# Darkkey/erlamsa

Measured on AMD Instinct MI355X. Metric: mutated_MB_per_s, higher is better.
Workload: dtype u8 (byte edits) + f64 (AS183 draws)

## Files before the change

erlamsa_amd/csrc/eh_device.h:

```cpp
#pragma once
#include <hip/hip_runtime.h>
#include <stdint.h>

#include "eh_common.h"

namespace eh {

#define EH_LANE ((int)threadIdx.x)
#define EH_DEV __device__ __forceinline__

EH_DEV uint32_t uni(uint32_t v) { return (uint32_t)__builtin_amdgcn_readfirstlane((int)v); }
EH_DEV uint64_t uni64(uint64_t v) { return ((uint64_t)uni((uint32_t)(v >> 32)) << 32) | uni((uint32_t)v); }
EH_DEV void wave_sync() { __syncthreads(); }

struct alignas(16) TabU16x65 { uint16_t v[65]; };
constexpr TabU16x65 as183_powers(uint32_t mult, uint32_t prime) {
  TabU16x65 t{};
  uint32_t a = 1;
  for (int k = 0; k <= 64; k++) { t.v[k] = (uint16_t)a; a = a * mult % prime; }
  return t;
}
__constant__ TabU16x65 c_T1 = as183_powers(171, 30269);
__constant__ TabU16x65 c_T2 = as183_powers(172, 30307);
__constant__ TabU16x65 c_T3 = as183_powers(170, 30323);
// ... 238 lines not shown
  bptr trace;
  uint32_t ntrace, tr_base;
  uint32_t co_posted;
  int32_t call_req, mu_phase, call_nres, call_nfs;
  uint64_t call_bin; uint32_t call_len;
  EH_G MuFrame* mu;
  uint64_t t_case;
  int32_t m_aux;
  uint64_t ws_peak, ws_top;
  int status;
  int lastm;
  uint64_t work;
  int r_kind;
  bptr r_ptr;
  uint32_t r_len;
  int r_flush;
  int r_drop_next;
  int r_changed;
  int r2; bptr r2_ptr; uint32_t r2_len;
  int nfs;
  uint64_t work_budget;
  uint64_t ovf_need, ovf_req;
  int ovf_line;
  int depth;
  int gen_pending;
  uint32_t gen_e1, gen_e2;
  int pat_ret; uint32_t pat_ip; int pat_cont;
  uint32_t fp_on, fp_g, fp_special, fp_keypos, fp_bA, fp_bB;
};
__shared__ Ctx g_ctx;
#ifdef HIPEMU
#define EH_LDS_ARRAY(type, name, n) static type name[n]
#define EH_KEEP(v) do {} while (0)
#else
#define EH_LDS_ARRAY(type, name, n) __shared__ type name[n]
#define EH_KEEP(v) asm volatile("" : "+v"(v))
#endif
EH_DEV void lanes_sync() { (void)__ballot(1); }
#define EH_CTX Ctx& c = g_ctx
#ifndef EH_FUSE_LDS_WORDS
#define EH_FUSE_LDS_WORDS 4800
#endif
EH_LDS_ARRAY(uint32_t, g_fuse_lds, EH_FUSE_LDS_WORDS);
EH_LDS_ARRAY(uint32_t, g_st_save, ST_STATE_WORDS);
struct LaneTab {
  uint32_t e_pri;
  uint32_t e_meta;
};
enum { R_SAME = 0, R_NEW = 1 };

#ifdef EH_PROF
#define EH_PT0 uint64_t pt_ = __builtin_readcyclecounter()
#define EH_PT(c, k) do { uint64_t n_ = __builtin_readcyclecounter(); if (EH_LANE == 0) { atomicAdd(&(c).p->prof[2 * (k)], (unsigned long long)(n_ - pt_)); atomicAdd(&(c).p->prof[2 * (k) + 1], 1ull); } pt_ = n_; } while (0)
#else
#define EH_PT0 do {} while (0)
#define EH_PT(c, k) do {} while (0)
#endif

EH_DEV void tr_b(Ctx& c, uint32_t v) {
  if (c.ntrace < TRACE_CAP - 1) { if (EH_LANE == 0) c.trace[c.ntrace] = (uint8_t)v; c.ntrace++; }
  else { if (EH_LANE == 0) c.trace[TRACE_CAP - 1] = 0xFF; c.ntrace = TRACE_CAP; }
}
EH_DEV void tr_v(Ctx& c, uint64_t v) { while (v >= 128) { tr_b(c, (uint32_t)(v & 127u) | 128u); v >>= 7; } tr_b(c, (uint32_t)v); }
__device__ __noinline__ void tr_aa_emit(int a, int b) { Ctx& c = g_ctx; tr_b(c, TRK_AA); tr_b(c, (uint32_t)a); tr_b(c, (uint32_t)b); }
__device__ __noinline__ void tr_ai_emit(int a, int64_t v) { Ctx& c = g_ctx; tr_b(c, TRK_AI); tr_b(c, (uint32_t)a); tr_v(c, ((uint64_t)v << 1) ^ (uint64_t)(v >> 63)); }
__device__ __noinline__ void tr_kv_emit(int kind, int nb, uint32_t b0, uint32_t b1, int nv, uint64_t v0, uint64_t v1, uint64_t v2) {
  Ctx& c = g_ctx;
  tr_b(c, (uint32_t)kind);
  if (nb > 0) tr_b(c, b0);
  if (nb > 1) tr_b(c, b1);
  if (nv > 0) tr_v(c, v0);
  if (nv > 1) tr_v(c, v1);
  if (nv > 2) tr_v(c, v2);
}
__device__ __noinline__ void tr_name_emit(cbptr nm, uint32_t nl, uint32_t up) {
  Ctx& c = g_ctx;
  tr_b(c, TRK_ARCHIVER); tr_v(c, nl + 3u * up);
  for (uint32_t k = 0; k < up; k++) { tr_b(c, '.'); tr_b(c, '.'); tr_b(c, '/'); }
  for (uint32_t k = 0; k < nl; k++) tr_b(c, uni(nm[k]));
}
EH_DEV void tr_aa(Ctx& c, int a, int b) { if (__builtin_expect(c.trace != nullptr, 0)) tr_aa_emit(a, b); }
EH_DEV void tr_ai(Ctx& c, int a, int64_t v) { if (__builtin_expect(c.trace != nullptr, 0)) tr_ai_emit(a, v); }
EH_DEV void tr_drop_before(Ctx& c, uint32_t start) {
  if (!c.trace || start <= c.tr_base || c.ntrace >= TRACE_CAP) return;
  const uint32_t n = c.ntrace - start;
  wave_sync();
  if (n) wave_move_down(c.trace + c.tr_base, c.trace + start, n);
  wave_sync();
  c.ntrace = c.tr_base + n;
}

EH_DEV void pool_nap() {
#ifndef HIPEMU
  __builtin_amdgcn_s_sleep(64);
#else
  fprintf(stderr, "hipemu: a wait for a pool area can never end with one wavefront running (block %u)\n", blockIdx.x); abort();
#endif
}
EH_DEV uint32_t pool_pop(const EH_G KParams& p, int t) {
  uint32_t v = 0xFFFFFFFFu;
  if (EH_LANE == 0) {
    unsigned long long h = atomicAdd(&p.pool_ctr[2 * t], 1ull);
    wptr e = p.pool_ring[t] + (h % p.pool_cnt[t]);
    v = atomicExch(e, 0xFFFFFFFFu);
    if (v == 0xFFFFFFFFu) {
      uint64_t w0 = __builtin_readcyclecounter();
      for (;;) { pool_nap(); v = atomicExch(e, 0xFFFFFFFFu); if (v != 0xFFFFFFFFu) break; }
      atomicAdd(&p.pool_ctr[20 + t], (unsigned long long)(__builtin_readcyclecounter() - w0));
      atomicAdd(&p.pool_ctr[30 + t], 1ull);
// ... 789 lines not shown
```

erlamsa_amd/csrc/eh_fuse.h:

```cpp
#pragma once
#include "eh_field.h"

namespace eh {

struct FNode { uint32_t fo, fc, to, tc; };

EH_DEV uint32_t wave_sort64(uint32_t key) {
  const uint32_t l = (uint32_t)EH_LANE;
#pragma unroll
  for (uint32_t k2 = 2; k2 <= 64; k2 <<= 1) {
#pragma unroll
    for (uint32_t j = k2 >> 1; j > 0; j >>= 1) {
      uint32_t other = (uint32_t)__shfl_xor((int)key, (int)j);
      bool up = (l & k2) == 0 || k2 == 64, lower = (l & j) == 0;
      bool take_min = lower == up;
      uint32_t mn = key < other ? key : other, mx = key < other ? other : key;
      key = take_min ? mn : mx;
    }
  }
  return key;
}
EH_DEV uint32_t lanes_le(uint32_t v, uint32_t cnt, uint32_t x) {
  uint32_t lo = 0;
#pragma unroll
// ... 231 lines not shown
    if (child) {
      FNode c2;
      c2.fc = nf; c2.tc = nt;
      c2.fo = special ? la : (nf == 1 ? fsurv + 1 : of);
      c2.to = special ? lb : (nt == 1 ? tsurv + 1 : (nt == 0 ? 0u : ot));
      o.nd[oc] = c2;
      le += nf + nt;
    }
    {
      bool lmulti = __shfl((int)(child && !special && nf > 1 ? 1 : 0), (int)lead[0]) != 0;
      uint32_t lof = (uint32_t)__shfl((int)of, (int)lead[0]);
      bool ldrop = __shfl((int)(isdrop[0] ? 1 : 0), (int)lead[0]) != 0;
      if (alive[0] && lmulti && !isdrop[0]) o.F[lof + ((uint32_t)l - lead[0]) - (ldrop ? 1u : 0u)] = pos[0] + 1;
    }
    if (!sym) {
      uint32_t sl = lanes_lt(gk[0], totf, gk[1]);
      uint32_t sk_at = (uint32_t)__shfl((int)gk[0], (int)(sl & 63));
      bool has = alive[1] && sl < totf && sk_at == gk[1];
      bool smulti = __shfl((int)(child && !special && nt > 1 ? 1 : 0), (int)(sl & 63)) != 0;
      uint32_t sot = (uint32_t)__shfl((int)ot, (int)(sl & 63));
      bool ldrop = __shfl((int)(isdrop[1] ? 1 : 0), (int)lead[1]) != 0;
      if (has && smulti && !isdrop[1]) o.T[sot + ((uint32_t)l - lead[1]) - (ldrop ? 1u : 0u)] = pos[1] + 1;
    }
    cn += (uint32_t)__builtin_amdgcn_readlane((int)ic, 63); cf += (uint32_t)__builtin_amdgcn_readlane((int)iff, 63); ct += (uint32_t)__builtin_amdgcn_readlane((int)it, 63);
    k0 += nfit;
  }
  *entries = wave_sum64(le);
  wave_sync();
  return cn;
}

__device__ bool fuse_jump_stream(Ctx& c, cbptr A, uint32_t la, cbptr B, uint32_t lb, bool sym, uint32_t* from, uint32_t* tpos, uint32_t* rounds);
}
#include "eh_fuse_red.h"
namespace eh {

#ifdef EH_FUSE_INLINE
EH_DEV bool fuse_lists(Ctx& c, cbptr A, uint32_t la, cbptr B, uint32_t lb, bptr* out, uint32_t* outlen) {
#else
__device__ __noinline__ bool fuse_lists(Ctx&, cbptr A, uint32_t la, cbptr B, uint32_t lb, bptr* out, uint32_t* outlen) {
  EH_CTX;
#endif
  const int l = EH_LANE;
  if (la == 0) { *out = (bptr)B; *outlen = lb; return true; }
  if (lb == 0) { *out = (bptr)A; *outlen = la; return true; }
  uint64_t mark = c.ws_used;
  const bool sym = A == B && la == lb;
  EH_PT0;
  uint32_t from = la, tpos = lb;
  uint32_t prof_rounds = 0;
  c.fp_on = 0;
  if ((sym ? (uint64_t)la : (uint64_t)la + lb) > FL_NMAX && !c.work_budget && !(c.p->flags & EH_FLAG_FUSE_NO_REDUCE)) {
    const uint32_t rd = fr_peek_rounds(c.rng);
    if (rd < 64) {
      const uint32_t R = rd + 2u;
      uint32_t la2 = la, lb2 = lb;
      cbptr A2 = fr_reduce(c, A, &la2, R);
      if (!A2) return false;
      cbptr B2 = A2;
      if (sym) lb2 = la2; else { B2 = fr_reduce(c, B, &lb2, R); if (!B2) return false; }
      if ((uint64_t)la2 + lb2 <= ((uint64_t)la + lb) / 4u * 3u) {
        EH_PT(c, 97);
        c.fp_on = 1;
        bool ok;
        if ((sym ? (uint64_t)la2 : (uint64_t)la2 + lb2) <= FL_NMAX && !(c.p->flags & EH_FLAG_FUSE_NO_LDS)) ok = fuse_jump_lds(c, A2, la2, B2, lb2, sym, &from, &tpos, &prof_rounds);
        else ok = fuse_jump_stream(c, A2, la2, B2, lb2, sym, &from, &tpos, &prof_rounds);
        c.fp_on = 0;
        if (!ok) return false;
        EH_PT(c, 54);
        const uint32_t g = c.fp_g, par = g & 1u;
        from = la; tpos = lb;
        if (g == 0) { from = rng_rand(c.rng, la); tpos = rng_rand(c.rng, lb); }
        else if (c.fp_special) { (void)rng_rand(c.rng, 1); (void)rng_rand(c.rng, 1); }
        else {
          cbptr key = A2 + c.fp_keypos;
          const uint32_t limA = la > g ? la - g : 0u, limB = lb > g ? lb - g : 0u;
          const uint32_t fc0 = fr_occ(A, la, limA, key, g, FR_NONE, nullptr), fc = fc0 + c.fp_bA;
          uint32_t pos = 0;
          if (fc > 0) { uint32_t j = rng_rand(c.rng, fc); j = par ? fc - 1u - j : j; if (j < fc0) { (void)fr_occ(A, la, limA, key, g, j, &pos); from = uni(pos) + g; } }
          const uint32_t tc0 = sym ? fc0 : fr_occ(B, lb, limB, key, g, FR_NONE, nullptr), tc = tc0 + c.fp_bB;
          if (tc > 0) { uint32_t j = rng_rand(c.rng, tc); j = par ? tc - 1u - j : j; if (j < tc0) { (void)fr_occ(B, lb, limB, key, g, j, &pos); tpos = uni(pos) + g; } }
        }
        EH_PT(c, 55);
        goto jump;
      }
    }
    EH_PT(c, 98);
    c.ws_used = mark;
  }
  if ((sym ? (uint64_t)la : (uint64_t)la + lb) <= FL_NMAX && !(c.p->flags & EH_FLAG_FUSE_NO_LDS)) {
    if (!fuse_jump_lds(c, A, la, B, lb, sym, &from, &tpos, &prof_rounds)) { if (c.status == CASE_BUDGET) c.ws_used = mark; return false; }
  } else if ((uint64_t)la + lb >= c.p->fuse_stream_min) {
    if (!fuse_jump_stream(c, A, la, B, lb, sym, &from, &tpos, &prof_rounds)) { if (c.status == CASE_BUDGET) c.ws_used = mark; return false; }
  } else {
    FuseGen g[2];
    for (int k = 0; k < 2; k++) {
      g[k].nd = (EH_G FNode*)ws_alloc(c, ((uint64_t)la + 4) * sizeof(FNode));
      g[k].F = (wptr)ws_alloc(c, ((uint64_t)la + 4) * 4);
      g[k].T = sym ? g[k].F : (wptr)ws_alloc(c, ((uint64_t)lb + 4) * 4);
      if (!g[k].nd || !g[k].F || !g[k].T) return false;
    }
    if (la > 1) for (uint32_t i = l; i < la; i += 64) g[0].F[i] = i;
    if (lb > 1 && !sym) for (uint32_t i = l; i < lb; i += 64) g[0].T[i] = i;
    if (l == 0) { FNode n0; n0.fo = 0; n0.fc = la; n0.to = 0; n0.tc = lb; g[0].nd[0] = n0; }
    uint32_t nn = 1, par = 0;
    int64_t fuel = 100000;
    uint64_t gen_entries = (uint64_t)la + lb;
    wave_sync();
    while (true) {
      if (fuel < 0) break;
      if (rng_rand(c.rng, 8) == 0) break;
      if (c.work_budget) {
        c.work += 16ull * gen_entries;
        if (c.work > c.work_budget) { c.status = CASE_BUDGET; c.ws_used = mark; return false; }
      }
      uint32_t nchild = fuse_round(A, la, B, lb, g[par], nn, g[par ^ 1], par, sym, &gen_entries);
      if (nchild == 0) break;
      par ^= 1; nn = nchild;
      fuel -= (int64_t)nchild;
      prof_rounds++;
    }
    uint32_t ni = rng_rand(c.rng, nn);
    FNode nd = g[par].nd[par ? nn - 1 - ni : ni];
    uint32_t fo = uni(nd.fo), fc = uni(nd.fc), to = sym ? fo : uni(nd.to), tc = sym ? fc : uni(nd.tc);
    if (fc > 0) { uint32_t j = rng_rand(c.rng, fc); from = fc == 1 ? fo : uni(g[par].F[fo + (par ? fc - 1 - j : j)]); }
    if (tc > 0) { uint32_t j = rng_rand(c.rng, tc); tpos = tc == 1 ? to : uni(g[par].T[to + (par ? tc - 1 - j : j)]); }
  }
jump:
#ifdef EH_PROF
  {
    uint32_t tot = la + lb, b = 0; while ((256u << b) < tot && b < 13) b++;
    EH_PT(c, 112 + b);
    if (EH_LANE == 0) { atomicAdd(&c.p->prof[2 * 126], (unsigned long long)prof_rounds); atomicAdd(&c.p->prof[2 * 126 + 1], 1ull); }
  }
#endif
  c.ws_used = mark;
  uint32_t nl = from + (lb - tpos);
  bptr dst = ws_alloc(c, nl);
// ... 50 lines not shown
```

erlamsa_amd/csrc/eh_fuse_lds.h:

```cpp
#pragma once

namespace eh {

constexpr uint32_t FL_NMAX = 8192;
constexpr uint32_t FL_E_WORDS = FL_NMAX / 2;
constexpr uint32_t FL_M_OFF = FL_E_WORDS, FL_M_WORDS = 264;
constexpr uint32_t FL_H_OFF = FL_M_OFF + FL_M_WORDS, FL_H_WORDS = 264;
constexpr uint32_t FL_NONE = 0xFFFFFFFFu;
static_assert(FL_H_OFF + FL_H_WORDS <= EH_FUSE_LDS_WORDS, "g_fuse_lds too small for eh_fuse_lds.h");
constexpr uint32_t FL_CUR = 0x3FFFu, FL_DEAD = 1u << 14, FL_DROPA = 1u << 15, FL_DROPB = 1u << 30, FL_SP = 1u << 31;

struct FlState {
  cbptr A; cbptr B; uint32_t la, lb; bool sym;
  uint32_t n, g, nn;
  uint32_t ghost;
  uint32_t nsp;
  uint32_t multi;
  uint32_t dboff;
  wptr T;
  uint32_t fast, tab_g0, ntomb;
};
struct FlRound { uint32_t w, nn, ghost, nsp, multi; };

EH_DEV uint16_t* fl_E() { return reinterpret_cast<uint16_t*>(g_fuse_lds); }
EH_DEV uint32_t* fl_M() { return g_fuse_lds + FL_M_OFF; }
EH_DEV uint32_t* fl_H() { return g_fuse_lds + FL_H_OFF; }

EH_DEV uint32_t fl_byte(const FlState& st, uint32_t e, bool side, uint32_t s) {
  uint32_t b;
  if (st.dboff != FL_NONE) b = reinterpret_cast<const uint8_t*>(g_fuse_lds)[st.dboff + e + st.g];
  else b = side ? st.B[s + st.g] : st.A[s + st.g];
  return (st.g & 1u) ? 255u - b : b;
}
EH_DEV uint64_t fl_window(uint32_t i, uint32_t* b64) {
  const uint32_t* M = fl_M();
  uint32_t w0 = M[i >> 5], w1 = M[(i >> 5) + 1], w2 = M[(i >> 5) + 2], sh = i & 31u;
  uint64_t lo = ((uint64_t)w1 << 32) | w0;
  uint64_t r = sh ? (lo >> sh) | ((uint64_t)w2 << (64 - sh)) : lo;
  *b64 = sh ? (w2 >> sh) & 1u : w2 & 1u;
  return r;
}
EH_DEV uint32_t fl_next_start(uint32_t j, uint32_t n) {
  const uint32_t* M = fl_M();
  const uint32_t l = (uint32_t)EH_LANE;
  for (uint32_t wbase = j >> 5; wbase * 32u < n; wbase += 64) {
    uint32_t wd = wbase + l;
    uint32_t v = wd * 32u < n ? M[wd] : 0u;
    if (wd == (j >> 5)) v &= ~0u << (j & 31u);
    unsigned long long any = __ballot(v != 0);
    if (any) {
      int src = (int)__builtin_ctzll(any);
      uint32_t vv = (uint32_t)__builtin_amdgcn_readlane((int)v, src);
      uint32_t idx = (wbase + (uint32_t)src) * 32u + (uint32_t)__builtin_ctz(vv);
      return idx < n ? idx : n;
    }
  }
  return n;
}
EH_DEV uint32_t fl_kth_start(uint32_t k, uint32_t n) {
  const uint32_t* M = fl_M();
  const uint32_t l = (uint32_t)EH_LANE;
  uint32_t seen = 0;
  for (uint32_t wbase = 0; wbase * 32u < n; wbase += 64) {
    uint32_t wd = wbase + l;
    uint32_t v = wd * 32u < n ? M[wd] : 0u;
    if (wd * 32u + 32u > n && wd * 32u < n) v &= (1u << (n & 31u)) - 1u;
    uint32_t c = (uint32_t)__popc(v);
    uint32_t inc = wave_incl_scan(c);
    uint32_t tot = (uint32_t)__builtin_amdgcn_readlane((int)inc, 63);
    if (seen + tot > k) {
      unsigned long long hit = __ballot(seen + inc > k);
      int src = (int)__builtin_ctzll(hit);
      uint32_t vv = (uint32_t)__builtin_amdgcn_readlane((int)v, src);
      uint32_t before = seen + (uint32_t)__builtin_amdgcn_readlane((int)(inc - c), src);
      uint32_t r = k - before;
      for (uint32_t t = 0; t < r; t++) vv &= vv - 1u;
      return (wbase + (uint32_t)src) * 32u + (uint32_t)__builtin_ctz(vv);
    }
    seen += tot;
  }
  return n;
}
EH_DEV void fl_clear_bits(uint32_t a, uint32_t b) {
// ... 225 lines not shown
      lanes_sync();
      for (uint32_t base = 0; base < st.n; base += 64) {
        uint32_t e = base + l < st.n ? (uint32_t)E[base + l] : 0xFFFFu;
        uint32_t d = st.la - st.g - e;
        if (e != 0xFFFFu && d < 64u) H[d] = base + l;
      }
      lanes_sync();
    }
    const uint32_t at = st.g <= st.la ? H[st.g - st.tab_g0] : FL_NONE;
    if (at == FL_NONE) { st.g++; return st.nn; }
    if (st.nn == 1) return 0;
    if (l == 0) { E[at] = 0xFFFFu; H[64u + st.ntomb] = at; }
    lanes_sync();
    st.ntomb++; st.nn--; st.g++;
    return st.nn;
  }
  uint32_t i = 0;
  while (i < st.n) {
    uint32_t b64 = 0;
    uint64_t sb = fl_window(i, &b64);
    uint32_t rest = st.n - i;
    uint32_t m;
    if (rest <= 64) m = rest;
    else {
      uint64_t cand = (sb >> 1) | ((uint64_t)b64 << 63);
      m = cand ? 64u - (uint32_t)__builtin_clzll(cand) : 0u;
    }
    if (rest < 64) sb &= (1ull << rest) - 1ull;
    if (m == 0) {
      uint32_t end = fl_next_start(i + 65, st.n);
      fl_big(st, i, end - i, o);
      i = end;
    } else {
      if (m < 64) sb &= (1ull << m) - 1ull;
      const uint64_t ones = m < 64 ? (1ull << m) - 1ull : ~0ull;
      if (st.sym && sb == ones) fl_singles(st, i, m, o);
      else fl_chunk(st, i, m, sb, o);
      i += m;
    }
  }
  if (o.nn == 0) return 0;
  st.n = o.w; st.nn = o.nn; st.ghost = o.ghost; st.nsp = o.nsp; st.multi = o.multi; st.g++;
  return o.nn;
}

__device__ __noinline__ bool fuse_jump_lds(Ctx&, cbptr A, uint32_t la, cbptr B, uint32_t lb, bool sym, uint32_t* from, uint32_t* tpos, uint32_t* rounds) {
  EH_CTX;
  const uint32_t l = (uint32_t)EH_LANE;
  FlState st;
  st.A = A; st.B = B; st.la = la; st.lb = lb; st.sym = sym;
  const uint32_t n0 = sym ? la : la + lb;
  st.n = n0; st.g = 0; st.nn = 1; st.ghost = FL_NONE; st.nsp = 0; st.multi = n0 > 1 ? 1u : 0u; st.dboff = FL_NONE;
  st.fast = 0; st.tab_g0 = 0; st.ntomb = 0;
  st.T = nullptr;
  if (n0 > 64) { st.T = (wptr)ws_alloc(c, 4ull * n0); if (!st.T) return false; }
  uint16_t* E = fl_E();
  for (uint32_t k = l; k < n0; k += 64) E[k] = (uint16_t)k;
  for (uint32_t k = l; k < FL_M_WORDS; k += 64) fl_M()[k] = k == 0 ? 1u : 0u;
  {
    uint32_t dbytes = sym ? la : la + lb, off = (2u * n0 + 15u) & ~15u;
    if (off + dbytes + 16u <= FL_E_WORDS * 4u) {
      uint8_t* D = reinterpret_cast<uint8_t*>(g_fuse_lds) + off;
      for (uint32_t k = l; k < la; k += 64) D[k] = A[k];
      if (!sym) for (uint32_t k = l; k < lb; k += 64) D[la + k] = B[k];
      st.dboff = off;
    }
  }
  lanes_sync();
  EH_PT0;
  int64_t fuel = 100000;
  uint64_t gen_entries = (uint64_t)la + lb;
  while (true) {
    if (fuel < 0) break;
    if (rng_rand(c.rng, 8) == 0) break;
    if (c.work_budget) {
      c.work += 16ull * gen_entries;
      if (c.work > c.work_budget) { c.status = CASE_BUDGET; return false; }
    }
#ifdef EH_PROF
    const int pslot = (st.sym && st.multi == 0) ? 102 : (st.g == 0 ? 100 : 101);
#endif
    uint32_t nchild = fl_round(st);
    EH_PT(c, pslot);
    if (nchild == 0) break;
    fuel -= (int64_t)nchild;
    gen_entries = sym ? 2ull * (st.n - st.ntomb) : (uint64_t)st.n + st.nsp;
    (*rounds)++;
  }
  const uint32_t par = st.g & 1u;
  uint32_t ni = rng_rand(c.rng, st.nn);
  uint32_t k = par ? st.nn - 1u - ni : ni;
  uint32_t a, b;
  if (st.sym && st.multi == 0) {
    a = k;
    if (st.ntomb) {
      const uint32_t* H = fl_H();
      for (;;) {
        uint32_t cdead = 0;
        for (uint32_t t0 = 0; t0 < st.ntomb; t0 += 64) cdead += (uint32_t)__popcll(__ballot(t0 + l < st.ntomb && H[64u + t0 + l] <= a));
        if (k + cdead == a) break;
        a = k + cdead;
      }
    }
    b = a + 1u;
  } else { a = fl_kth_start(k, st.n); b = fl_next_start(a + 1u, st.n); }
  uint32_t fc = b - a;
  if (!sym) {
    uint32_t cnt = 0;
    for (uint32_t base = a; base < b; base += 64) cnt += (uint32_t)__popcll(__ballot(base + l < b && (uint32_t)E[base + l] < la));
    fc = cnt;
  }
  uint32_t tc = sym ? fc : (b - a) - fc;
  if (c.fp_on) {
    const uint32_t e0 = uni((uint32_t)E[a]), el = uni((uint32_t)E[a + fc - 1u]);
    c.fp_g = st.g; c.fp_keypos = e0;
    c.fp_special = (fc == 1u && e0 + st.g == la) ? 1u : 0u;
    c.fp_bA = (el + st.g == la) ? 1u : 0u;
    c.fp_bB = sym ? c.fp_bA : ((tc > 0 && uni((uint32_t)E[b - 1u]) - la + st.g == lb) ? 1u : 0u);
    EH_PT(c, 103);
    return true;
  }
  bool special_t = false;
  if (!sym && tc == 0 && a != st.ghost) { tc = 1; special_t = true; }
  *from = la; *tpos = lb;
  if (fc > 0) { uint32_t j = rng_rand(c.rng, fc); *from = (uint32_t)E[a + (par ? fc - 1u - j : j)] + st.g; }
  if (tc > 0) {
    uint32_t j = rng_rand(c.rng, tc);
    if (!special_t) { uint32_t idx = sym ? a + (par ? tc - 1u - j : j) : a + fc + (par ? tc - 1u - j : j); uint32_t e = (uint32_t)E[idx]; *tpos = (sym ? e : e - la) + st.g; }
  }
  *from = uni(*from); *tpos = uni(*tpos);
  EH_PT(c, 103);
  return true;
}

// ... 2 lines not shown
```

erlamsa_amd/csrc/eh_fuse_red.h:

```cpp
#pragma once

namespace eh {

constexpr uint32_t FR_NONE = 0xFFFFFFFFu;
constexpr uint32_t FR_MAX_PERIOD = 1u << 16;
constexpr int FR_LEVELS = 4;

EH_DEV uint64_t fr_ld8(cbptr S, uint32_t q, uint32_t len) {
  uint64_t by = 0;
  if (q + 8 <= len) by = ldg8(S + q);
  else { for (uint32_t k = 0; k < 8; k++) if (q + k < len) by |= (uint64_t)S[q + k] << (8 * k); }
  return by;
}
EH_DEV uint32_t fr_peek_rounds(const Rng& r) {
  const uint32_t l = (uint32_t)EH_LANE;
  double x = rng_peek(r, l + 1u) * 8.0;
  unsigned long long z = __ballot((uint32_t)x == 0u);
  return z ? (uint32_t)__builtin_ctzll(z) : 64u;
}
__device__ __noinline__ uint32_t fr_run_fwd(cbptr S, uint32_t i0, uint32_t p, uint32_t n) {
  const uint32_t l = (uint32_t)EH_LANE;
  const uint32_t lim = n - p;
  for (uint32_t base = i0;; base += 1024) {
    const uint32_t q = base + 16u * l;
// ... 110 lines not shown
  const uint32_t l = (uint32_t)EH_LANE;
  uint64_t k8 = 0;
  for (uint32_t k = 0; k < 8 && k < g; k++) k8 |= (uint64_t)key[k] << (8 * k);
  const uint64_t mask = g >= 8 ? ~0ull : ((1ull << (8 * g)) - 1ull);
  uint32_t seen = 0;
  for (uint32_t base = 0; base < lim; base += 4096) {
    uint64_t lo[4], hi[4], nx[4];
#pragma unroll
    for (int u = 0; u < 4; u++) {
      const uint32_t s0 = base + 1024u * (uint32_t)u + 16u * l;
      lo[u] = hi[u] = nx[u] = 0;
      if (s0 < lim) {
        if (s0 + 24 <= len) { const uint4 v = ldg16(S + s0); lo[u] = (uint64_t)v.x | ((uint64_t)v.y << 32); hi[u] = (uint64_t)v.z | ((uint64_t)v.w << 32); nx[u] = ldg8(S + s0 + 16); }
        else { lo[u] = fr_ld8(S, s0, len); hi[u] = fr_ld8(S, s0 + 8, len); nx[u] = fr_ld8(S, s0 + 16, len); }
      }
    }
#pragma unroll
    for (int u = 0; u < 4; u++) {
      const uint32_t s0 = base + 1024u * (uint32_t)u + 16u * l;
      uint32_t bits = 0;
#pragma unroll
      for (uint32_t k = 0; k < 16; k++) {
        const uint64_t a = k < 8 ? lo[u] : hi[u], b = k < 8 ? hi[u] : nx[u];
        const uint32_t sh = 8u * (k & 7u);
        const uint64_t w = sh ? (a >> sh) | (b << (64u - sh)) : a;
        if ((w & mask) == k8 && s0 + k < lim) bits |= 1u << k;
      }
      if (g > 8 && __ballot(bits != 0)) {
        uint32_t left = bits;
        while (left) {
          const uint32_t k = (uint32_t)__builtin_ctz(left); left &= left - 1u;
          const uint32_t s = s0 + k;
          for (uint32_t q = 8; q < g; q++) if (S[s + q] != key[q]) { bits &= ~(1u << k); break; }
        }
      }
      const uint32_t cnt = (uint32_t)__popc(bits);
      const uint32_t inc = wave_incl_scan(cnt);
      const uint32_t tot = (uint32_t)__builtin_amdgcn_readlane((int)inc, 63);
      if (want != FR_NONE && want < seen + tot) {
        const uint32_t r = want - seen, ex = inc - cnt;
        const bool mine = r >= ex && r < inc;
        uint32_t p = 0;
        if (mine) { uint32_t b = bits; for (uint32_t t = ex; t < r; t++) b &= b - 1u; p = s0 + (uint32_t)__builtin_ctz(b); }
        const unsigned long long who = __ballot(mine);
        *pos = (uint32_t)__builtin_amdgcn_readlane((int)p, (int)__builtin_ctzll(who));
        return seen + tot;
      }
      seen += tot;
    }
  }
  return seen;
}

}
```

erlamsa_amd/engine.py:

```python
import ctypes as C
import os

import numpy as np

_HERE = os.path.dirname(os.path.abspath(__file__))
LIB_PATH = os.environ.get("ERLAMSA_HIP_LIB") or os.path.join(_HERE, "liberlamsa_hip.so")

EH_ABI_VERSION = 8
EH_FLAG_ORDERED_OUTPUT = 1
EH_FLAG_META_TRACE = 2
EH_FLAG_FUSE_NO_LDS = 4
EH_FLAG_FUSE_NO_REDUCE = 8
EH_FLAG_SGML_NO_REPLAY = 16
EH_FLAG_SGML_NO_LANES = 32
EH_FLAG_NO_COOP = 64

UNIQUE_PIECE_BYTES = 65536

CASE_OK, CASE_CRASHED, CASE_OVERFLOW, CASE_UNSUPPORTED, CASE_ARENA_FULL, CASE_BUDGET = 0, 1, 2, 3, 4, 5

ABI_SYMBOLS = [
    "eh_create", "eh_destroy", "eh_configure", "eh_corpus_upload", "eh_corpus_attach", "eh_fuzz_batch",
    "eh_fuzz_calls", "eh_reserve", "eh_sync", "eh_result_device", "eh_result_download", "eh_result_fetch", "eh_result_totals", "eh_result_summary", "eh_result_occupancy", "eh_result_diag", "eh_result_cycles", "eh_result_peak", "eh_result_meta", "eh_result_write_files", "eh_result_prof", "eh_selftest_movers", "eh_selftest_zlib",
    "eh_last_kernel_ms", "eh_pool_stats", "eh_coop_stats", "eh_kernel_name", "eh_abi_version", "eh_mutator_count", "eh_mutator_name",
    "eh_mutator_default_pri", "eh_mutator_on_gpu", "eh_pattern_count", "eh_pattern_name",
    "eh_pattern_default_pri", "eh_pattern_on_gpu", "eh_strerror", "eh_last_error",
    "eh_coalesce_limits", "eh_submit", "eh_flush", "eh_poll", "eh_cancel",
    "eh_corpus_device", "eh_stream", "eh_host_alloc", "eh_host_free", "eh_selftest_sort_by_priority", "eh_last_error_copy",
    "eh_comm_unique_id", "eh_comm_init", "eh_comm_init_local", "eh_comm_destroy", "eh_corpus_broadcast", "eh_corpus_allgather",
    "eh_corpus_broadcast_local", "eh_device_count", "eh_meta_atom_count", "eh_meta_atom_name", "eh_batch_done",
    "eh_result_digests", "eh_result_unique", "eh_result_download_select", "eh_selftest_unique",
]


class EhOptions(C.Structure):
    _fields_ = [("abi_version", C.c_uint32), ("mutations", C.c_char_p), ("patterns", C.c_char_p),
                ("generators", C.c_char_p), ("blockscale", C.c_double), ("ssrf_host", C.c_char_p),
                ("ssrf_port", C.c_int32), ("max_case_bytes", C.c_uint64), ("out_capacity", C.c_uint64),
                ("max_case_work", C.c_uint64), ("max_slots", C.c_uint32), ("flags", C.c_uint32), ("big_case_bytes", C.c_uint64),
                ("pool_bytes", C.c_uint64), ("download_chunk_bytes", C.c_uint64), ("fuse_stream_min", C.c_uint64),
                ("sequence_muta", C.c_uint32), ("reserved0", C.c_uint32)]


class EngineError(RuntimeError):
    def __init__(self, code, msg):
        super().__init__("erlamsa_hip error %d: %s" % (code, msg))
        self.code = code


_lib = None


def load_library():
    global _lib
    if _lib is not None:
        return _lib
    import sys
    if "torch" in sys.modules:
        import torch
        if torch.cuda.is_available():
            torch.cuda.init()
    if not os.path.exists(LIB_PATH):
        raise ImportError("%s not built: run `python -c 'import __graft_entry__ as g; g.build()'`" % LIB_PATH)
    lib = C.CDLL(LIB_PATH)
    vp, u64p, i64p, i32p = C.c_void_p, C.POINTER(C.c_uint64), C.POINTER(C.c_int64), C.POINTER(C.c_int32)
# ... 474 lines not shown
```

include/erlamsa_hip.h:

```cpp
#ifndef ERLAMSA_HIP_H
#define ERLAMSA_HIP_H
#include <stdint.h>
#ifdef __cplusplus
extern "C" {
#endif

#define EH_ABI_VERSION 8

typedef struct eh_ctx eh_ctx;

enum eh_error {
  EH_OK = 0,
  EH_E_INVALID = -1,
  EH_E_NODEVICE = -2,
  EH_E_HIP = -3,
  EH_E_NOMEM = -4,
  EH_E_STATE = -5,
  EH_E_UNSUPPORTED = -6,
  EH_E_AGAIN = -7
};

enum eh_case_status {
  EH_CASE_OK = 0,
  EH_CASE_CRASHED = 1,
  EH_CASE_OVERFLOW = 2,
  EH_CASE_UNSUPPORTED = 3,
  EH_CASE_ARENA_FULL = 4,
  EH_CASE_BUDGET = 5
};

typedef struct eh_options {
  uint32_t abi_version;
  const char* mutations;
  const char* patterns;
  const char* generators;
  double blockscale;
  const char* ssrf_host;
  int32_t ssrf_port;
  uint64_t max_case_bytes;
  uint64_t out_capacity;
  uint64_t max_case_work;
  uint32_t max_slots;
  uint32_t flags;
  uint64_t big_case_bytes;
  uint64_t pool_bytes;
  uint64_t download_chunk_bytes;
  uint64_t fuse_stream_min;
  uint32_t sequence_muta;
  uint32_t reserved0;
} eh_options;

#define EH_FLAG_NO_COOP 64u
#define EH_FLAG_TREE_NO_LANES 128u
#define EH_FLAG_ORDERED_OUTPUT 1u
#define EH_FLAG_META_TRACE 2u
#define EH_FLAG_SGML_NO_LANES 32u
#define EH_FLAG_SGML_NO_REPLAY 16u
#define EH_FLAG_FUSE_NO_REDUCE 8u
#define EH_FLAG_FUSE_NO_LDS 4u

int eh_create(int device, eh_ctx** out);
void eh_destroy(eh_ctx* ctx);
int eh_configure(eh_ctx* ctx, const eh_options* opts);

int eh_corpus_upload(eh_ctx* ctx, const uint8_t* data, const uint64_t* off, uint64_t n);
int eh_corpus_attach(eh_ctx* ctx, const void* d_data, const void* d_off, uint64_t n, uint64_t nbytes);

int eh_device_count(void);
int eh_comm_unique_id(uint8_t id[128]);
int eh_comm_init(eh_ctx* ctx, const uint8_t id[128], int rank, int nranks);
int eh_comm_init_local(eh_ctx** ctxs, int nctx);
int eh_comm_destroy(eh_ctx* ctx);
int eh_corpus_broadcast(eh_ctx* ctx, int root, const uint8_t* data, const uint64_t* off, uint64_t n);
int eh_corpus_allgather(eh_ctx* ctx, const uint8_t* data, const uint64_t* off, uint64_t n_local);
int eh_corpus_broadcast_local(eh_ctx** ctxs, int nctx, int root);

int eh_corpus_device(eh_ctx* ctx, const void** d_data, const void** d_off, uint64_t* n, uint64_t* nbytes);

int eh_stream(eh_ctx* ctx, void** stream);

int eh_host_alloc(void** p, uint64_t bytes);
void eh_host_free(void* p);

int eh_reserve(eh_ctx* ctx, uint64_t max_cases);

int eh_fuzz_batch(eh_ctx* ctx, const int64_t seed[3], uint64_t first_case, uint64_t corpus_first, uint64_t n,
                  void* stream);
int eh_fuzz_calls(eh_ctx* ctx, const int64_t* seeds, uint64_t corpus_first, uint64_t n, void* stream);
int eh_sync(eh_ctx* ctx);
int eh_batch_done(eh_ctx* ctx, int* done);

int eh_coalesce_limits(eh_ctx* ctx, uint64_t flush_cases, uint64_t flush_bytes);
int eh_submit(eh_ctx* ctx, const uint8_t* data, uint64_t len, const int64_t seed[3], uint64_t* ticket);
int eh_flush(eh_ctx* ctx);
int eh_poll(eh_ctx* ctx, uint64_t ticket, uint8_t* out, uint64_t cap, uint64_t* out_len, int32_t* status);
int eh_cancel(eh_ctx* ctx, uint64_t ticket);

int eh_result_device(eh_ctx* ctx, const uint8_t** d_data, const uint64_t** d_off, const uint64_t** d_len,
                     const int32_t** d_status, uint64_t* total_bytes);
int eh_result_download(eh_ctx* ctx, uint8_t* data, uint64_t cap, uint64_t* off, int32_t* status);
int eh_result_fetch(eh_ctx* ctx, uint64_t i, uint8_t* buf, uint64_t cap, uint64_t* out_len);
int eh_result_totals(eh_ctx* ctx, uint64_t* in_bytes, uint64_t* out_bytes, uint64_t* n_cases);
int eh_result_summary(eh_ctx* ctx, uint64_t* out);
int eh_result_occupancy(eh_ctx* ctx, uint64_t* out);
int eh_result_diag(eh_ctx* ctx, uint64_t* draws, int32_t* last_mutator);

// ... 49 lines not shown
```

Baseline: 79880.

## Add hash-based R-gram dedup path before LDS suffix-jump in fuse

For large fuse inputs, a new pre-pass hashes every R-byte window into a global open-addressing table and keeps one representative position per distinct window. The deduplicated positions are transposed into a per-depth strided byte plane, so the LDS fuse path can run on a much smaller set. Each round stages that plane into LDS. The goal is to stop falling back to the slower reduce/stream paths on inputs longer than the LDS capacity. The cost is an extra hashing pass, table clearing and workspace use, and it relies on atomics to keep the minimum position per slot. The new path is on by default and can be disabled with a new flag.

Measured after the change: 79980 (median of 2 runs). No clear change (+0.1%).

```diff
diff --git a/erlamsa_amd/csrc/eh_device.h b/erlamsa_amd/csrc/eh_device.h
--- a/erlamsa_amd/csrc/eh_device.h
+++ b/erlamsa_amd/csrc/eh_device.h
@@ -314,9 +314,11 @@
 #ifdef EH_PROF
 #define EH_PT0 uint64_t pt_ = __builtin_readcyclecounter()
 #define EH_PT(c, k) do { uint64_t n_ = __builtin_readcyclecounter(); if (EH_LANE == 0) { atomicAdd(&(c).p->prof[2 * (k)], (unsigned long long)(n_ - pt_)); atomicAdd(&(c).p->prof[2 * (k) + 1], 1ull); } pt_ = n_; } while (0)
+#define EH_PT_RESTART do { pt_ = __builtin_readcyclecounter(); } while (0)
 #else
 #define EH_PT0 do {} while (0)
 #define EH_PT(c, k) do {} while (0)
+#define EH_PT_RESTART do {} while (0)
 #endif
 
 EH_DEV void tr_b(Ctx& c, uint32_t v) {
diff --git a/erlamsa_amd/csrc/eh_fuse.h b/erlamsa_amd/csrc/eh_fuse.h
--- a/erlamsa_amd/csrc/eh_fuse.h
+++ b/erlamsa_amd/csrc/eh_fuse.h
@@ -307,7 +307,34 @@
   c.fp_on = 0;
   if ((sym ? (uint64_t)la : (uint64_t)la + lb) > FL_NMAX && !c.work_budget && !(c.p->flags & EH_FLAG_FUSE_NO_REDUCE)) {
     const uint32_t rd = fr_peek_rounds(c.rng);
-    if (rd < 64) {
+    cbptr key = nullptr;
+    bool named = false;
+    if (rd < 64 && !(c.p->flags & (EH_FLAG_FUSE_NO_DEDUP | EH_FLAG_FUSE_NO_LDS))) {
+      const uint32_t R = rd + 2u;
+      FD_COUNT(4);
+      if (R > FD_RCAP) FD_COUNT(FD_OVER_CAP);
+      else {
+        const uint64_t rc = fr_dedup(c, A, la, B, lb, sym, R);
+        if (rc == FD_NOMEM) return false;
+        if (rc > FD_NOMEM) {
+          cbptr W = (cbptr)rc + FD_W_OFF;
+          FD_COUNT(0);
+          EH_PT_RESTART;
+          c.fp_on = 2;
+          const bool ok = fuse_jump_lds(c, W, c.fp_bA, W, c.fp_bB, sym, &from, &tpos, &prof_rounds);
+          c.fp_on = 0;
+          if (!ok) return false;
+          EH_PT(c, 43);
+          key = A + uni(((cwptr)rc)[c.fp_keypos]);
+          named = true;
+        } else {
+          FD_COUNT((uint32_t)rc);
+          EH_PT(c, 44);
+          c.ws_used = mark;
+        }
+      }
+    }
+    if (!named && rd < 64) {
       const uint32_t R = rd + 2u;
       uint32_t la2 = la, lb2 = lb;
       cbptr A2 = fr_reduce(c, A, &la2, R);
@@ -323,12 +350,16 @@
         c.fp_on = 0;
         if (!ok) return false;
         EH_PT(c, 54);
+        key = A2 + c.fp_keypos;
+        named = true;
+      }
+    }
+    if (named) {
         const uint32_t g = c.fp_g, par = g & 1u;
         from = la; tpos = lb;
         if (g == 0) { from = rng_rand(c.rng, la); tpos = rng_rand(c.rng, lb); }
         else if (c.fp_special) { (void)rng_rand(c.rng, 1); (void)rng_rand(c.rng, 1); }
         else {
-          cbptr key = A2 + c.fp_keypos;
           const uint32_t limA = la > g ? la - g : 0u, limB = lb > g ? lb - g : 0u;
           const uint32_t fc0 = fr_occ(A, la, limA, key, g, FR_NONE, nullptr), fc = fc0 + c.fp_bA;
           uint32_t pos = 0;
@@ -338,7 +369,6 @@
         }
         EH_PT(c, 55);
         goto jump;
-      }
     }
     EH_PT(c, 98);
     c.ws_used = mark;
diff --git a/erlamsa_amd/csrc/eh_fuse_lds.h b/erlamsa_amd/csrc/eh_fuse_lds.h
--- a/erlamsa_amd/csrc/eh_fuse_lds.h
+++ b/erlamsa_amd/csrc/eh_fuse_lds.h
@@ -17,6 +17,7 @@
   uint32_t nsp;
   uint32_t multi;
   uint32_t dboff;
+  uint32_t pstride;
   wptr T;
   uint32_t fast, tab_g0, ntomb;
 };
@@ -28,7 +29,8 @@
 
 EH_DEV uint32_t fl_byte(const FlState& st, uint32_t e, bool side, uint32_t s) {
   uint32_t b;
-  if (st.dboff != FL_NONE) b = reinterpret_cast<const uint8_t*>(g_fuse_lds)[st.dboff + e + st.g];
+  if (st.pstride != FL_NONE) b = st.dboff != FL_NONE ? reinterpret_cast<const uint8_t*>(g_fuse_lds)[st.dboff + e] : st.A[st.g * st.pstride + e];
+  else if (st.dboff != FL_NONE) b = reinterpret_cast<const uint8_t*>(g_fuse_lds)[st.dboff + e + st.g];
   else b = side ? st.B[s + st.g] : st.A[s + st.g];
   return (st.g & 1u) ? 255u - b : b;
 }
@@ -360,12 +362,15 @@
   const uint32_t n0 = sym ? la : la + lb;
   st.n = n0; st.g = 0; st.nn = 1; st.ghost = FL_NONE; st.nsp = 0; st.multi = n0 > 1 ? 1u : 0u; st.dboff = FL_NONE;
   st.fast = 0; st.tab_g0 = 0; st.ntomb = 0;
+  st.pstride = c.fp_on == 2u ? ((n0 + 15u) & ~15u) : FL_NONE;
   st.T = nullptr;
   if (n0 > 64) { st.T = (wptr)ws_alloc(c, 4ull * n0); if (!st.T) return false; }
   uint16_t* E = fl_E();
   for (uint32_t k = l; k < n0; k += 64) E[k] = (uint16_t)k;
   for (uint32_t k = l; k < FL_M_WORDS; k += 64) fl_M()[k] = k == 0 ? 1u : 0u;
-  {
+  const uint32_t stage = (2u * n0 + 15u) & ~15u;
+  const bool stage_fits = st.pstride != FL_NONE && stage + st.pstride <= FL_E_WORDS * 4u;
+  if (st.pstride == FL_NONE) {
     uint32_t dbytes = sym ? la : la + lb, off = (2u * n0 + 15u) & ~15u;
     if (off + dbytes + 16u <= FL_E_WORDS * 4u) {
       uint8_t* D = reinterpret_cast<uint8_t*>(g_fuse_lds) + off;
@@ -388,6 +393,13 @@
 #ifdef EH_PROF
     const int pslot = (st.sym && st.multi == 0) ? 102 : (st.g == 0 ? 100 : 101);
 #endif
+    if (stage_fits && !(st.sym && st.multi == 0)) {
+      uint32_t* D = g_fuse_lds + (stage >> 2);
+      lanes_sync();
+      for (uint32_t k = l; k < (st.pstride >> 4); k += 64) { const uint4 v = ldg16(st.A + (uint64_t)st.g * st.pstride + 16u * k); D[4 * k] = v.x; D[4 * k + 1] = v.y; D[4 * k + 2] = v.z; D[4 * k + 3] = v.w; }
+      st.dboff = stage;
+      lanes_sync();
+    }
     uint32_t nchild = fl_round(st);
     EH_PT(c, pslot);
     if (nchild == 0) break;
diff --git a/erlamsa_amd/csrc/eh_fuse_red.h b/erlamsa_amd/csrc/eh_fuse_red.h
--- a/erlamsa_amd/csrc/eh_fuse_red.h
+++ b/erlamsa_amd/csrc/eh_fuse_red.h
@@ -186,4 +186,181 @@
   return seen;
 }
 
-}
+#ifndef EH_FD_RCAP
+#define EH_FD_RCAP 32
+#endif
+constexpr uint32_t FD_RCAP = EH_FD_RCAP;
+static_assert(FD_RCAP >= 2 && FD_RCAP <= 32, "EH_FD_RCAP: 2 .. 32");
+constexpr uint32_t FD_TBL_BITS = 15, FD_TBL = 1u << FD_TBL_BITS;
+#if defined(HIPEMU) && defined(EH_FD_HASH_BITS)
+constexpr uint32_t FD_HASH_MASK = (1u << EH_FD_HASH_BITS) - 1u, FD_PROBES = 2048;
+#else
+constexpr uint32_t FD_HASH_MASK = FD_TBL - 1u, FD_PROBES = 64;
+#endif
+constexpr uint32_t FD_MUL = 0x01000193u;
+enum : uint32_t { FD_OK = 0, FD_OVER_CAP = 1, FD_OVER_NMAX = 2, FD_TABLE_FULL = 3, FD_NOMEM = 4 };
+#ifdef HIPEMU
+extern "C" { inline unsigned long long eh_emu_fuse_dedup[5] = {0, 0, 0, 0, 0}; }
+#define FD_COUNT(i) do { if (EH_LANE == 0) eh_emu_fuse_dedup[i] += 1; } while (0)
+#else
+#define FD_COUNT(i) do { } while (0)
+#endif
+
+EH_DEV uint32_t fd_ld(cwptr p) { return __atomic_load_n(p, __ATOMIC_RELAXED); }
+EH_DEV uint4 fd_ld16(cbptr S, uint32_t q, uint32_t len) {
+  if (q + 16 <= len) return ldg16(S + q);
+  uint32_t w[4] = {0, 0, 0, 0};
+#pragma unroll
+  for (uint32_t k = 0; k < 16; k++) if (q + k < len) w[k >> 2] |= (uint32_t)S[q + k] << (8 * (k & 3));
+  uint4 r; r.x = w[0]; r.y = w[1]; r.z = w[2]; r.w = w[3];
+  return r;
+}
+EH_DEV bool fd_same(cbptr S, uint32_t len, uint32_t a, uint32_t b, uint32_t from, uint32_t R) {
+  for (uint32_t j = from; j < R; j += 8) {
+    uint64_t x = fr_ld8(S, a + j, len) ^ fr_ld8(S, b + j, len);
+    if (R - j < 8) x &= (1ull << (8 * (R - j))) - 1ull;
+    if (x) return false;
+  }
+  return true;
+}
+EH_DEV uint32_t fd_slot(uint32_t h) { return ((h * 0x9E3779B1u) >> (32 - FD_TBL_BITS)) & FD_HASH_MASK; }
+EH_DEV uint32_t fd_insert(cbptr S, uint32_t len, uint32_t R, wptr T, uint32_t p) {
+  uint32_t h = 0;
+  for (uint32_t j = 0; j < R; j++) h = h * FD_MUL + (uint32_t)S[p + j];
+  uint32_t slot = fd_slot(h);
+  for (uint32_t t = 0; t < FD_PROBES; t++) {
+    uint32_t cur = fd_ld(&T[slot]);
+    if (cur == FR_NONE) { cur = atomicCAS(&T[slot], FR_NONE, p); if (cur == FR_NONE) return 1u; }
+    if (fd_same(S, len, cur, p, 0, R)) { if (p < cur) (void)atomicMin(&T[slot], p); return 0u; }
+    slot = (slot + 1u) & (FD_TBL - 1u);
+  }
+  return FD_PROBES + 1u;
+}
+__device__ __noinline__ uint32_t fd_pass_a(cbptr S, uint32_t len, uint32_t lim, uint32_t R, wptr T, uint32_t budget) {
+  const uint32_t l = (uint32_t)EH_LANE;
+  uint32_t pw = 1;
+  for (uint32_t k = 1; k < R; k++) pw *= FD_MUL;
+  const uint64_t m0 = R >= 8 ? ~0ull : ((1ull << (8 * R)) - 1ull);
+  const uint64_t m1 = R >= 16 ? ~0ull : (R > 8 ? ((1ull << (8 * (R - 8))) - 1ull) : 0ull);
+  uint32_t total = 0;
+  uint4 n0 = fd_ld16(S, 16u * l, len), n1 = fd_ld16(S, 16u * l + 16u, len), nin = fd_ld16(S, 16u * l + R, len);
+  for (uint32_t base = 0; base < lim; base += 1024) {
+    const uint32_t q = base + 16u * l;
+    const uint4 v0 = n0, v1 = n1, vin = nin;
+    if (base + 1024 < lim) { const uint32_t q2 = q + 1024u; n0 = fd_ld16(S, q2, len); n1 = fd_ld16(S, q2 + 16u, len); nin = fd_ld16(S, q2 + R, len); }
+    const uint32_t b32[8] = {v0.x, v0.y, v0.z, v0.w, v1.x, v1.y, v1.z, v1.w}, in32[4] = {vin.x, vin.y, vin.z, vin.w};
+    uint32_t h = 0, slot[16];
+#pragma unroll
+    for (uint32_t k = 0; k < 32; k++) if (k < R) h = h * FD_MUL + ((b32[k >> 2] >> (8 * (k & 3))) & 255u);
+#pragma unroll
+    for (uint32_t k = 0; k < 16; k++) {
+      slot[k] = fd_slot(h);
+      h = (h - ((b32[k >> 2] >> (8 * (k & 3))) & 255u) * pw) * FD_MUL + ((in32[k >> 2] >> (8 * (k & 3))) & 255u);
+    }
+    uint32_t cur[16];
+#pragma unroll
+    for (uint32_t k = 0; k < 16; k++) cur[k] = q + k < lim ? fd_ld(&T[slot[k]]) : FR_NONE;
+    uint64_t c0[16], c1[16];
+#pragma unroll
+    for (uint32_t k = 0; k < 16; k++) {
+      c0[k] = c1[k] = 0;
+      if (cur[k] != FR_NONE) { c0[k] = fr_ld8(S, cur[k], len); if (R > 8) c1[k] = fr_ld8(S, cur[k] + 8u, len); }
+    }
+    const uint64_t d[4] = {(uint64_t)v0.x | ((uint64_t)v0.y << 32), (uint64_t)v0.z | ((uint64_t)v0.w << 32), (uint64_t)v1.x | ((uint64_t)v1.y << 32), (uint64_t)v1.z | ((uint64_t)v1.w << 32)};
+    uint32_t need = 0;
+#pragma unroll
+    for (uint32_t k = 0; k < 16; k++) {
+      const uint32_t sh = 8u * (k & 7u), p = q + k;
+      const uint64_t w0 = sh ? (d[k >> 3] >> sh) | (d[(k >> 3) + 1] << (64u - sh)) : d[k >> 3];
+      const uint64_t w1 = sh ? (d[(k >> 3) + 1] >> sh) | (d[(k >> 3) + 2] << (64u - sh)) : d[(k >> 3) + 1];
+      if (p < lim) {
+        bool same = cur[k] != FR_NONE && ((c0[k] ^ w0) & m0) == 0 && ((c1[k] ^ w1) & m1) == 0;
+        if (same && R > 16) same = fd_same(S, len, cur[k], p, 16, R);
+        if (same) { if (p < cur[k]) (void)atomicMin(&T[slot[k]], p); }
+        else need |= 1u << k;
+      }
+    }
+    uint32_t ins = 0;
+    while (need) { const uint32_t k = (uint32_t)__builtin_ctz(need); need &= need - 1u; ins += fd_insert(S, len, R, T, q + k); if (ins > FD_PROBES) break; }
+    if (__ballot(ins > FD_PROBES) != 0) return FD_TABLE_FULL << 28;
+    total += wave_sum(ins);
+    if (total > budget) return FD_OVER_NMAX << 28;
+  }
+  return total;
+}
+EH_DEV uint32_t fd_side(Ctx& c, cbptr S, uint32_t len, uint32_t R, wptr T, uint32_t budget, wptr P) {
+  const uint32_t l = (uint32_t)EH_LANE;
+  if (len <= FL_NMAX / 4u || len <= R) {
+    if (len > budget) return FD_OVER_NMAX << 28;
+    for (uint32_t i = l; i < len; i += 64) P[i] = i;
+    return len;
+  }
+  if (R > budget) return FD_OVER_NMAX << 28;
+  const uint32_t lim = len - R, nw = (lim + 31u) >> 5;
+  const uint64_t mark = c.ws_used;
+  wptr BM = (wptr)ws_alloc(c, 4ull * nw);
+  if (!BM) return FD_NOMEM << 28;
+  { uint4 none; none.x = none.y = none.z = none.w = FR_NONE; for (uint32_t i = l; i < FD_TBL / 4u; i += 64) stg16a(T + 4u * i, none); }
+  for (uint32_t i = l; i < nw; i += 64) BM[i] = 0;
+  wave_sync();
+  EH_PT0;
+  const uint32_t rc = fd_pass_a(S, len, lim, R, T, budget - R);
+  wave_sync();
+  EH_PT(c, 41);
+  if (rc >> 28) { c.ws_used = mark; return rc; }
+  for (uint32_t i = l; i < FD_TBL; i += 256) {
+    uint32_t v[4];
+#pragma unroll
+    for (uint32_t u = 0; u < 4; u++) v[u] = fd_ld(&T[i + 64u * u]);
+#pragma unroll
+    for (uint32_t u = 0; u < 4; u++) if (v[u] != FR_NONE) (void)atomicOr(&BM[v[u] >> 5], 1u << (v[u] & 31u));
+  }
+  wave_sync();
+  uint32_t w = 0;
+  for (uint32_t base = 0; base < nw; base += 64) {
+    uint32_t bits = base + l < nw ? fd_ld(&BM[base + l]) : 0u;
+    const uint32_t cnt = (uint32_t)__popc(bits), inc = wave_incl_scan(cnt);
+    uint32_t at = w + inc - cnt;
+    while (bits) { if (at < budget) P[at] = (base + l) * 32u + (uint32_t)__builtin_ctz(bits); at++; bits &= bits - 1u; }
+    w += (uint32_t)__builtin_amdgcn_readlane((int)inc, 63);
+  }
+  c.ws_used = mark;
+  if (w + R > budget) return FD_OVER_NMAX << 28;
+  for (uint32_t j = l; j < R; j += 64) P[w + j] = lim + j;
+  return w + R;
+}
+constexpr uint32_t FD_W_OFF = 4u * FL_NMAX;
+__device__ __noinline__ uint64_t fr_dedup(Ctx&, cbptr A, uint32_t la, cbptr B, uint32_t lb, bool sym, uint32_t R) {
+  EH_CTX;
+  const uint32_t l = (uint32_t)EH_LANE;
+  bptr buf = ws_alloc(c, (uint64_t)FD_W_OFF + (uint64_t)R * FL_NMAX);
+  if (!buf) return FD_NOMEM;
+  wptr P = (wptr)buf;
+  bptr W = buf + FD_W_OFF;
+  const uint64_t mark = c.ws_used;
+  wptr T = (wptr)ws_alloc(c, 4ull * FD_TBL);
+  if (!T) return FD_NOMEM;
+  uint32_t KA = fd_side(c, A, la, R, T, FL_NMAX, P), KB = 0;
+  if (KA >> 28) return KA >> 28;
+  if (!sym) { KB = fd_side(c, B, lb, R, T, FL_NMAX - KA, P + KA); if (KB >> 28) return KB >> 28; }
+  c.ws_used = mark;
+  EH_PT0;
+  const uint32_t n0 = sym ? KA : KA + KB, stride = (n0 + 15u) & ~15u;
+  wave_sync();
+  for (uint32_t e = l; e < n0; e += 64) {
+    const bool side = e >= KA;
+    cbptr S = side ? B : A;
+    const uint32_t len = side ? lb : la, pos = P[e];
+    for (uint32_t g0 = 0; g0 < R; g0 += 8) {
+      const uint64_t x = fr_ld8(S, pos + g0, len);
+#pragma unroll
+      for (uint32_t j = 0; j < 8; j++) if (g0 + j < R) W[(uint64_t)(g0 + j) * stride + e] = (uint8_t)(x >> (8 * j));
+    }
+  }
+  wave_sync();
+  EH_PT(c, 42);
+  c.fp_bA = KA; c.fp_bB = sym ? KA : KB;
+  return (uint64_t)buf;
+}
+
+}
diff --git a/erlamsa_amd/engine.py b/erlamsa_amd/engine.py
--- a/erlamsa_amd/engine.py
+++ b/erlamsa_amd/engine.py
@@ -11,6 +11,7 @@
 EH_FLAG_META_TRACE = 2
 EH_FLAG_FUSE_NO_LDS = 4
 EH_FLAG_FUSE_NO_REDUCE = 8
+EH_FLAG_FUSE_NO_DEDUP = 256
 EH_FLAG_SGML_NO_REPLAY = 16
 EH_FLAG_SGML_NO_LANES = 32
 EH_FLAG_NO_COOP = 64
diff --git a/include/erlamsa_hip.h b/include/erlamsa_hip.h
--- a/include/erlamsa_hip.h
+++ b/include/erlamsa_hip.h
@@ -52,6 +52,7 @@
 
 #define EH_FLAG_NO_COOP 64u
 #define EH_FLAG_TREE_NO_LANES 128u
+#define EH_FLAG_FUSE_NO_DEDUP 256u
 #define EH_FLAG_ORDERED_OUTPUT 1u
 #define EH_FLAG_META_TRACE 2u
 #define EH_FLAG_SGML_NO_LANES 32u
```
